# VisualComputingInstitute/diffusion-e2e-ft

Measured on NVIDIA H100. Metric: images_per_sec_768x768_depth, higher is better.
Workload: dtype fp16

## Files before the change

diffusion_e2e_ft_b200/build.py:

```python
import hashlib
import os
import subprocess
import sys
from concurrent.futures import ThreadPoolExecutor

HERE = os.path.dirname(os.path.abspath(__file__))
CSRC = os.path.join(HERE, "csrc")
OUT = os.path.join(HERE, "libb200_e2eft.so")
OBJ = os.path.join(HERE, "build")
SOURCES = ["gemm_conv.cu", "attention.cu", "norm.cu", "elementwise.cu", "conv_small.cu", "loss.cu", "optim.cu", "backward.cu", "postproc.cu",
           "evaluation.cu", "data.cu"]
NVCC = os.environ.get("NVCC", "/usr/local/cuda/bin/nvcc")
FLAGS = ["-gencode", "arch=compute_90a,code=sm_90a", "-O3", "-lineinfo", "-std=c++17",
         "-Xcompiler", "-fPIC"]


def _digest():
    h = hashlib.sha256()
    for root in (CSRC, os.path.join(HERE, "..", "include")):
        for f in sorted(os.listdir(root)):
            if f.endswith((".cu", ".cuh", ".h")):
                h.update(open(os.path.join(root, f), "rb").read())
    h.update(" ".join(FLAGS).encode())
    return h.hexdigest()


def build(force=False, verbose=False):
    os.makedirs(OBJ, exist_ok=True)
    stamp = os.path.join(OBJ, "stamp")
    dg = _digest()
    if not force and os.path.exists(OUT) and os.path.exists(stamp) and open(stamp).read() == dg:
        return OUT
    if not os.path.exists(NVCC):
        raise RuntimeError(f"nvcc not found at {NVCC}; cannot build {OUT}")

    def cc(src):
        obj = os.path.join(OBJ, src.replace(".cu", ".o"))
        cmd = [NVCC, *FLAGS, "-c", os.path.join(CSRC, src), "-o", obj]
        if verbose:
            cmd.insert(1, "-Xptxas=-v")
        r = subprocess.run(cmd, capture_output=True, text=True)
        if r.returncode != 0:
            raise RuntimeError(f"nvcc failed for {src}:\n{r.stdout}\n{r.stderr}")
        if verbose:
            print(r.stderr)
        return obj

    with ThreadPoolExecutor(max_workers=4) as ex:
        objs = list(ex.map(cc, SOURCES))
    r = subprocess.run([NVCC, "-shared", "-o", OUT, *objs, "-lcudart"], capture_output=True, text=True)
    if r.returncode != 0:
        raise RuntimeError(f"link failed:\n{r.stdout}\n{r.stderr}")
    open(stamp, "w").write(dg)
    return OUT


if __name__ == "__main__":
    print(build(force="--force" in sys.argv, verbose="-v" in sys.argv))
```

diffusion_e2e_ft_b200/csrc/gemm_conv.cu:

```cuda
#include <cstdarg>
#include <cstdio>
#include <cstring>
#include <mutex>

#include "gemm_conv.cuh"
#include "../../include/b200_e2eft.h"

namespace b200 {

static thread_local char g_err[512] = "";
void set_last_error(const char* fmt, ...) {
  va_list ap;
  va_start(ap, fmt);
  vsnprintf(g_err, sizeof(g_err), fmt, ap);
  va_end(ap);
}
const char* last_error() { return g_err; }

typedef CUresult (*EncodeTiledFn)(CUtensorMap*, CUtensorMapDataType, cuuint32_t, void*,
                                  const cuuint64_t*, const cuuint64_t*, const cuuint32_t*,
                                  const cuuint32_t*, CUtensorMapInterleave, CUtensorMapSwizzle,
                                  CUtensorMapL2promotion, CUtensorMapFloatOOBfill);
static EncodeTiledFn get_encode() {
  static EncodeTiledFn fn = nullptr;
  static std::once_flag once;
  std::call_once(once, [] {
    void* p = nullptr;
    cudaDriverEntryPointQueryResult q;
    if (cudaGetDriverEntryPoint("cuTensorMapEncodeTiled", &p, cudaEnableDefault, &q) == cudaSuccess &&
        q == cudaDriverEntryPointSuccess)
      fn = reinterpret_cast<EncodeTiledFn>(p);
  });
  return fn;
}

int encode_tmap(CUtensorMap* out, const void* gptr, int rank, const uint64_t* dims,
                const uint64_t* strides_bytes, const uint32_t* box, const uint32_t* elem_strides,
                CUtensorMapDataType dtype) {
  EncodeTiledFn fn = get_encode();
  if (!fn) {
    set_last_error("cuTensorMapEncodeTiled entry point unavailable (no CUDA driver?)");
    return -2;
  }
  cuuint64_t d[5], s[4];
  cuuint32_t b[5], e[5];
  for (int i = 0; i < rank; ++i) {
    d[i] = dims[i];
    b[i] = box[i];
    e[i] = elem_strides ? elem_strides[i] : 1;
  }
  for (int i = 0; i < rank - 1; ++i) s[i] = strides_bytes[i];
  CUresult r = fn(out, dtype, (cuuint32_t)rank, const_cast<void*>(gptr), d, s, b, e,
                  CU_TENSOR_MAP_INTERLEAVE_NONE, CU_TENSOR_MAP_SWIZZLE_128B,
                  CU_TENSOR_MAP_L2_PROMOTION_L2_256B, CU_TENSOR_MAP_FLOAT_OOB_FILL_NONE);
  if (r != CUDA_SUCCESS) {
    set_last_error(
        "cuTensorMapEncodeTiled failed (%d): rank %d dims [%llu %llu %llu %llu] strides [%llu %llu %llu] "
        "box [%u %u %u %u] ptr %p",
        (int)r, rank, (unsigned long long)d[0], (unsigned long long)(rank > 1 ? d[1] : 0),
        (unsigned long long)(rank > 2 ? d[2] : 0), (unsigned long long)(rank > 3 ? d[3] : 0),
        (unsigned long long)s[0], (unsigned long long)(rank > 2 ? s[1] : 0),
        (unsigned long long)(rank > 3 ? s[2] : 0), b[0], rank > 1 ? b[1] : 0, rank > 2 ? b[2] : 0,
        rank > 3 ? b[3] : 0, gptr);
    return -3;
  }
  return 0;
}

int current_device() {
  int dev = 0;
  return cudaGetDevice(&dev) == cudaSuccess && dev >= 0 && dev < kMaxDevices ? dev : -1;
}

int sm_count() {
  static int n[kMaxDevices] = {0};
  const int dev = current_device();
  if (dev < 0) return 132;
  if (!n[dev]) {
    int v = 0;
    cudaDeviceGetAttribute(&v, cudaDevAttrMultiProcessorCount, dev);
    n[dev] = v > 0 ? v : 132;
  }
  return n[dev];
}

constexpr int kLastLaunchFields = 16;
static int g_last_launch[kLastLaunchFields] = {0};

template <int BN, typename OutT, bool SWAP, bool GEGLU = false, bool HALO = false, bool VEC = false>
static int launch_one(const CUtensorMap& a, const CUtensorMap& a2, const CUtensorMap& b,
                      const GemmParams& p, cudaStream_t st) {
  using S = GemmSmem<BN, SWAP, HALO>;
  static bool configured_dev[kMaxDevices] = {false};
  const int dev = current_device();
  bool& configured = configured_dev[dev < 0 ? 0 : dev];
  auto kern = gemm_conv_kernel<BN, OutT, SWAP, GEGLU, HALO, VEC>;
  if (!configured || dev < 0) {
    cudaError_t e = cudaFuncSetAttribute(kern, cudaFuncAttributeMaxDynamicSharedMemorySize, S::kTotalBytes);
    if (e != cudaSuccess) {
      set_last_error("cudaFuncSetAttribute(smem=%d): %s", S::kTotalBytes, cudaGetErrorString(e));
      return (int)e;
    }
    configured = true;
  }
  int tiles = p.batch * p.m_tiles * p.n_tiles;
  int grid = tiles < sm_count() ? tiles : sm_count();
  if (SWAP && p.chan_stats && p.n_tiles > 1 && grid > p.n_tiles) grid -= grid % p.n_tiles;
  {
    const int rec[kLastLaunchFields] = {p.conv, HALO, SWAP, BN, VEC, GEGLU, (int)std::is_same<OutT, float>::value,
                                        p.bw, p.bh, p.halo_n, p.tiles_w, p.tiles_h, p.m_tiles, p.n_tiles, grid,
                                        p.chan_stats != nullptr};
    memcpy(g_last_launch, rec, sizeof(rec));
  }
  kern<<<grid, kGemmThreads, S::kTotalBytes, st>>>(a, a2, b, p);
  B200_CHECK_LAUNCH("gemm_conv_kernel");
  return 0;
}

template <typename OutT>
static int launch_bn(int bn, bool swap, const CUtensorMap& a, const CUtensorMap& a2, const CUtensorMap& b,
                     const GemmParams& p, cudaStream_t st) {
  if (swap) {
    switch (bn) {
      case 64: return p.vec_ok ? launch_one<64, OutT, true, false, false, true>(a, a2, b, p, st)
                               : launch_one<64, OutT, true>(a, a2, b, p, st);
      case 128: return p.vec_ok ? launch_one<128, OutT, true, false, false, true>(a, a2, b, p, st)
                                : launch_one<128, OutT, true>(a, a2, b, p, st);
      case 256: return p.vec_ok ? launch_one<256, OutT, true, false, false, true>(a, a2, b, p, st)
                                : launch_one<256, OutT, true>(a, a2, b, p, st);
    }
  } else if (p.act == ACT_GEGLU) {
    if constexpr (std::is_same<OutT, __half>::value) {
      switch (bn) {
        case 64: return launch_one<64, OutT, false, true>(a, a2, b, p, st);
        case 128: return launch_one<128, OutT, false, true>(a, a2, b, p, st);
        case 160: return launch_one<160, OutT, false, true>(a, a2, b, p, st);
        case 256: return launch_one<256, OutT, false, true>(a, a2, b, p, st);
      }
    }
    set_last_error("GEGLU epilogue needs fp16 output and a tile width in {64,128,160,256} (got %d)", bn);
    return -1;
  } else {
    switch (bn) {
      case 32: return launch_one<32, OutT, false>(a, a2, b, p, st);
      case 64: return launch_one<64, OutT, false>(a, a2, b, p, st);
      case 128: return launch_one<128, OutT, false>(a, a2, b, p, st);
      case 160: return launch_one<160, OutT, false>(a, a2, b, p, st);
      case 256: return launch_one<256, OutT, false>(a, a2, b, p, st);
    }
  }
  set_last_error("unsupported tile width %d (swap=%d)", bn, (int)swap);
  return -1;
}

static double kblock_cycles(int n) { return n * 4.0 > 365.0 ? n * 4.0 : 365.0; }
static double tiles_cost(long long tiles, int n) {
  long long waves = (tiles + sm_count() - 1) / sm_count();
  return (double)waves * (kblock_cycles(n) + 40.0);
}

static int g_force_bn = 0;
static int g_debug = 0;
static int g_swap_mode = 1;
static int g_halo_mode = 1;
static int g_last_path = 0;

static bool pick_halo_tile(int Ho, int Wo, int* bw_out, int* bh_out) {
  double best = 0.0;
  int bbw = 0, bbh = 0;
  for (int bw = 8; bw <= 254 && bw <= Wo; ++bw) {
    for (int bh = 1; bh <= 32 && bh <= Ho; ++bh) {
      const int pitch = bw + 2;
      const int n = (pitch * bh + 63) / 64 * 64;
      if (n > 256) break;
      if ((bh + 2) * pitch + (n - pitch * bh) + 2 > kHaloMaxPatchPix) continue;
      const double ew = (double)Wo / ((double)((Wo + bw - 1) / bw) * bw);
      const double eh = (double)Ho / ((double)((Ho + bh - 1) / bh) * bh);
      double score = ew * eh * (double)(bw * bh) / n;
      score *= 0.9 + 0.1 * n / 256.0;
      score *= 1.0 - 0.03 * ((double)(bw + 2) * (bh + 2) / (bw * bh) - 1.0);
      if (score > best + 1e-9) { best = score; bbw = bw; bbh = bh; }
    }
  }
  *bw_out = bbw; *bh_out = bbh;
  return bbw != 0 && best >= 0.78;
}

}

using namespace b200;

extern "C" const char* b200_last_error_string(void) { return b200::last_error(); }
extern "C" void b200_debug_force_block_n(int bn) { b200::g_force_bn = bn; }
extern "C" void b200_debug_set_flags(int f) { b200::g_debug = f; }
extern "C" void b200_debug_set_swap(int m) { b200::g_swap_mode = m; }
extern "C" void b200_debug_set_halo(int m) { b200::g_halo_mode = m; }
extern "C" int b200_debug_last_path(void) { return b200::g_last_path; }
extern "C" int b200_debug_last_launch(int* out, int n) {
  if (!out || n <= 0) return kLastLaunchFields;
  const int k = n < kLastLaunchFields ? n : kLastLaunchFields;
  memcpy(out, b200::g_last_launch, k * sizeof(int));
  return kLastLaunchFields;
}
extern "C" int b200_abi_version(void) { return 17; }
extern "C" int b200_geglu_block_n(int N) {
  return (N % 160 == 0) ? 160 : (N % 256 == 0 ? 256 : (N % 128 == 0 ? 128 : (N % 64 == 0 ? 64 : 0)));
}

extern "C" int b200_linear(const void* A, long long lda, long long a_batch_stride, const void* W,
                           long long ldw, long long w_batch_stride, int M, int N, int K, int batch,
                           const float* bias, int bias_row, const void* residual, long long ld_res,
                           long long res_batch_stride, void* out, long long ldo,
                           long long out_batch_stride, int out_f32, int act, float alpha,
                           double* chan_stats, int rows_per_img, void* out2_f16, int res_mul, int a_mn, int w_mn,
                           long long bias_batch_stride, void* stream) {
  B200_CHECK_ARG(A && W && out, "b200_linear: null pointer");
  B200_CHECK_ARG(!(a_mn || w_mn) || act != ACT_GEGLU, "b200_linear: MN-major operands are not combined with GEGLU");
  B200_CHECK_ARG(M > 0 && N > 0 && K > 0 && batch > 0, "b200_linear: bad shape M=%d N=%d K=%d batch=%d", M, N, K, batch);
  B200_CHECK_ARG(lda % 8 == 0 && ldw % 8 == 0, "b200_linear: lda/ldw must be multiples of 8 elements (16 B)");
  B200_CHECK_ARG(((uintptr_t)A & 15) == 0 && ((uintptr_t)W & 15) == 0 && ((uintptr_t)out & 15) == 0,
                 "b200_linear: pointers must be 16-byte aligned");
  B200_CHECK_ARG(act != ACT_GEGLU || ldo % 8 == 0, "b200_linear: GEGLU needs ldo %% 8 == 0");
  B200_CHECK_ARG(act != ACT_GEGLU || (N % 16 == 0 && bias), "b200_linear: GEGLU needs bias and N%%16==0");
  B200_CHECK_ARG(batch == 1 || (a_batch_stride % 8 == 0 && (w_batch_stride % 8 == 0)),
                 "b200_linear: batch strides must be multiples of 8 elements");

  B200_CHECK_ARG(!chan_stats || (batch == 1 && rows_per_img > 0 && rows_per_img % 64 == 0 && M % rows_per_img == 0 &&
                                 act != ACT_GEGLU && !bias_row),
                 "b200_linear: chan_stats needs batch=1, rows_per_img %% 64 == 0, M %% rows_per_img == 0");
  B200_CHECK_ARG((long long)M * ldo < 0xFFFFFFFFll && (long long)M * (ld_res > 0 ? ld_res : 1) < 0xFFFFFFFFll,
                 "b200_linear: per-batch output larger than 2^32 elements");
  GemmParams p;
  memset(&p, 0, sizeof(p));
  p.M = M; p.N = N;
  p.num_k_blocks = (K + kBlockK - 1) / kBlockK;
  p.batch = batch;
  p.m_tiles = (M + kBlockM - 1) / kBlockM;
  p.a_batched = (a_batch_stride != 0 && batch > 1);
  p.b_batched = (w_batch_stride != 0 && batch > 1);
  const bool can_swap = g_swap_mode && N >= 128 && act != ACT_GEGLU && !bias_row;
  bool swap = false;
  int bn = 0;
  double best = 1e30;
  if (act == ACT_GEGLU) {
    bn = b200_geglu_block_n(N);
    B200_CHECK_ARG(bn != 0, "b200_linear: GEGLU N=%d not tileable", N);
  } else {
    const int nc[5] = {256, 160, 128, 64, 32};
    const bool normal_ok = !chan_stats || rows_per_img % kBlockM == 0;
    for (int i = 0; i < 5 && normal_ok; ++i) {
      if (g_force_bn && nc[i] != g_force_bn) continue;
      if (w_mn && nc[i] % 64 != 0) continue;
      double c = tiles_cost((long long)p.m_tiles * batch * ((N + nc[i] - 1) / nc[i]), nc[i]);
      if (c < best - 1e-9) { best = c; bn = nc[i]; swap = false; }
    }
    if (can_swap || (chan_stats && !normal_ok && N >= 128)) {
      const int pc[3] = {256, 128, 64};
      for (int i = 0; i < 3; ++i) {
        if (g_force_bn && pc[i] != g_force_bn) continue;
        if (chan_stats && rows_per_img % pc[i] != 0) continue;
        if (a_mn && pc[i] % 64 != 0) continue;
        double c = tiles_cost((long long)batch * ((M + pc[i] - 1) / pc[i]) * ((N + 127) / 128), pc[i]) * 0.85;
        if (c < best - 1e-9) { best = c; bn = pc[i]; swap = true; }
      }
    }
    B200_CHECK_ARG(bn != 0, "b200_linear: no tile shape for N=%d (forced %d)", N, g_force_bn);
  }
  if (swap) {
    p.m_tiles = (M + bn - 1) / bn;
    p.n_tiles = (N + 127) / 128;
  } else {
    p.n_tiles = (N + bn - 1) / bn;
  }
  p.out = out; p.ldo = ldo; p.out_batch_stride = out_batch_stride; p.out_f32 = out_f32;
  p.bias = bias; p.bias_row = bias_row;
  p.residual = residual; p.ld_res = ld_res; p.res_batch_stride = res_batch_stride; p.res_mul = res_mul;
  p.act = act; p.alpha = alpha; p.debug = g_debug;
  p.chan_stats = chan_stats; p.rows_per_img = rows_per_img; p.out2 = (__half*)out2_f16;
  p.act_mn = a_mn; p.w_mn = w_mn;
  p.bias_bs = bias_batch_stride;
  p.out_mul = 1;
  {
    const uintptr_t omask = out_f32 ? 15 : 7;
    p.vec_ok = swap && (chan_stats != nullptr || (g_debug & 128)) && !(g_debug & 64) && N % 4 == 0 && ldo % 4 == 0 &&
               out_batch_stride % 4 == 0 && ((uintptr_t)out & omask) == 0 &&
               (!residual || (ld_res % 4 == 0 && res_batch_stride % 4 == 0 && ((uintptr_t)residual & omask) == 0)) &&
               (!out2_f16 || ((uintptr_t)out2_f16 & 7) == 0);
  }

  CUtensorMap ta, tb;
  if (a_mn) {
    uint64_t dims[3] = {(uint64_t)M, (uint64_t)K, (uint64_t)(p.a_batched ? batch : 1)};
    uint64_t str[2] = {(uint64_t)lda * 2, (uint64_t)(p.a_batched ? a_batch_stride : (long long)K * lda) * 2};
    uint32_t box[3] = {64, kBlockK, 1};
    int r = encode_tmap(&ta, A, 3, dims, str, box, nullptr);
    if (r) return r;
  } else {
    uint64_t dims[3] = {(uint64_t)K, (uint64_t)M, (uint64_t)(p.a_batched ? batch : 1)};
    uint64_t str[2] = {(uint64_t)lda * 2, (uint64_t)(p.a_batched ? a_batch_stride : (long long)M * lda) * 2};
    uint32_t box[3] = {kBlockK, (uint32_t)(swap ? bn : kBlockM), 1};
    int r = encode_tmap(&ta, A, 3, dims, str, box, nullptr);
    if (r) return r;
  }
  if (w_mn) {
    uint64_t dims[3] = {(uint64_t)N, (uint64_t)K, (uint64_t)(p.b_batched ? batch : 1)};
    uint64_t str[2] = {(uint64_t)ldw * 2, (uint64_t)(p.b_batched ? w_batch_stride : (long long)K * ldw) * 2};
    uint32_t box[3] = {64, kBlockK, 1};
    int r = encode_tmap(&tb, W, 3, dims, str, box, nullptr);
    if (r) return r;
  } else {
    uint64_t dims[3] = {(uint64_t)K, (uint64_t)N, (uint64_t)(p.b_batched ? batch : 1)};
    uint64_t str[2] = {(uint64_t)ldw * 2, (uint64_t)(p.b_batched ? w_batch_stride : (long long)N * ldw) * 2};
    uint32_t box[3] = {kBlockK, (uint32_t)(swap ? kBlockM : bn), 1};
    int r = encode_tmap(&tb, W, 3, dims, str, box, nullptr);
    if (r) return r;
  }
  cudaStream_t st = (cudaStream_t)stream;
  return out_f32 ? launch_bn<float>(bn, swap, ta, ta, tb, p, st) : launch_bn<__half>(bn, swap, ta, ta, tb, p, st);
}

static double pick_patch(int Ho, int Wo, int stride, int target, int* bw_out, int* bh_out) {
  double best = -1;
  int bbw = 1, bbh = 1;
  for (int bw = 1; bw <= target && bw <= Wo; ++bw) {
    if (bw * stride > 256) break;
    int bh = target / bw;
    if (bh > Ho) bh = Ho;
    if (bh * stride > 256) bh = 256 / stride;
    if (bh < 1) continue;
    long long tw = (Wo + bw - 1) / bw, th = (Ho + bh - 1) / bh;
    double eff = (double)Ho * Wo / (double)(tw * th * target);
    if (eff > best + 1e-9 || (eff > best - 1e-9 && bw > bbw)) {
      best = eff; bbw = bw; bbh = bh;
    }
  }
  *bw_out = bbw; *bh_out = bbh;
  return best;
}

extern "C" int b200_conv2d_nhwc(const void* X, int NB, int H, int W, int Cin, const void* X2, int C2,
                                const void* Wp, int Cout, int num_taps, const int* tap_dy,
                                const int* tap_dx, int stride, int Ho, int Wo, int out_mul, int out_oy,
                                int out_ox, const float* bias, const float* rowvec,
                                long long ld_rowvec, const void* residual, void* out, int out_f32,
                                int out_nchw, int act, double* chan_stats, void* out2_f16, void* stream) {
  B200_CHECK_ARG(X && Wp && out, "b200_conv2d_nhwc: null pointer");
  B200_CHECK_ARG(Cin % 64 == 0, "b200_conv2d_nhwc: Cin=%d must be a multiple of 64 (use im2col path)", Cin);
  B200_CHECK_ARG(C2 % 64 == 0, "b200_conv2d_nhwc: C2=%d must be a multiple of 64", C2);
  B200_CHECK_ARG(num_taps >= 1 && num_taps <= kMaxTaps, "b200_conv2d_nhwc: num_taps=%d", num_taps);
  B200_CHECK_ARG(stride >= 1 && stride <= 2 && out_mul >= 1, "b200_conv2d_nhwc: stride=%d out_mul=%d", stride, out_mul);
  B200_CHECK_ARG(NB > 0 && H > 0 && W > 0 && Ho > 0 && Wo > 0 && Cout > 0, "b200_conv2d_nhwc: bad shape");
  B200_CHECK_ARG(((uintptr_t)X & 15) == 0 && ((uintptr_t)Wp & 15) == 0 && ((uintptr_t)out & 15) == 0,
                 "b200_conv2d_nhwc: pointers must be 16-byte aligned");
  B200_CHECK_ARG(act != ACT_GEGLU, "b200_conv2d_nhwc: GEGLU epilogue is linear-only");
  B200_CHECK_ARG(!out_nchw || (!residual && Cout <= 8), "b200_conv2d_nhwc: out_nchw needs Cout <= 8 and no residual");

  B200_CHECK_ARG((long long)NB * Ho * out_mul * Wo * out_mul * Cout < 0xFFFFFFFFll,
                 "b200_conv2d_nhwc: output larger than 2^32 elements");
  GemmParams p;
  memset(&p, 0, sizeof(p));
  p.conv = 1;
  p.N = Cout;
  p.batch = 1;
  p.Ho = Ho; p.Wo = Wo;
  const bool can_swap = g_swap_mode && Cout >= 128 && !out_nchw;
  {
    bool taps_ok = stride == 1 && Ho == H && Wo == W && !(X2 && out_mul != 1);
    for (int i = 0; i < num_taps && taps_ok; ++i)
      taps_ok = tap_dy[i] >= -1 && tap_dy[i] <= 1 && tap_dx[i] >= -1 && tap_dx[i] <= 1;
    int hbw = 0, hbh = 0;
    const bool epi_bound = out_f32 && residual && num_taps * Cin <= 1152 && !X2;
    const bool halo_vec = !(g_debug & 64) && (Cout % 4 == 0) && (!residual || ((uintptr_t)residual & 15) == 0) &&
                          (!out2_f16 || ((uintptr_t)out2_f16 & 7) == 0);
    if (can_swap && g_halo_mode && taps_ok && !g_force_bn && halo_vec && (!epi_bound || g_halo_mode == 2) &&
        pick_halo_tile(Ho, Wo, &hbw, &hbh)) {
      p.bw = hbw; p.bh = hbh;
      p.col_pitch = hbw + 2;
      p.halo_n = ((hbw + 2) * hbh + 63) / 64 * 64;
      p.tiles_w = (Wo + hbw - 1) / hbw;
      p.tiles_h = (Ho + hbh - 1) / hbh;
      p.m_tiles = NB * p.tiles_w * p.tiles_h;
      p.n_tiles = (Cout + 127) / 128;
      p.M = NB * Ho * Wo;
      p.cin_blocks = Cin / 64;
// ... 129 lines not shown
```

diffusion_e2e_ft_b200/lib.py:

```python
import ctypes
import os
from ctypes import c_char_p, c_double, c_float, c_int, c_longlong, c_void_p, POINTER

_HERE = os.path.dirname(os.path.abspath(__file__))
LIB_PATH = os.path.join(_HERE, "libb200_e2eft.so")

_lib = None
ABI_VERSION = 17

_P = c_void_p
_LL = c_longlong
_SIGS = {
    "b200_last_error_string": (c_char_p, []),
    "b200_abi_version": (c_int, []),
    "b200_debug_force_block_n": (None, [c_int]),
    "b200_debug_set_flags": (None, [c_int]),
    "b200_debug_set_swap": (None, [c_int]),
    "b200_debug_set_halo": (None, [c_int]),
    "b200_debug_last_path": (c_int, []),
    "b200_debug_last_launch": (c_int, [POINTER(c_int), c_int]),
    "b200_geglu_block_n": (c_int, [c_int]),
    "b200_linear": (c_int, [_P, _LL, _LL, _P, _LL, _LL, c_int, c_int, c_int, c_int, _P, c_int, _P, _LL, _LL,
                            _P, _LL, _LL, c_int, c_int, c_float, _P, c_int, _P, c_int, c_int, c_int, _LL, _P]),
    "b200_conv2d_nhwc": (c_int, [_P, c_int, c_int, c_int, c_int, _P, c_int, _P, c_int, c_int,
                                 POINTER(c_int), POINTER(c_int), c_int, c_int, c_int, c_int, c_int, c_int,
                                 _P, _P, _LL, _P, _P, c_int, c_int, c_int, _P, _P, _P]),
    "b200_conv3x3_small_cout": (c_int, [_P, c_int, c_int, c_int, c_int, _P, _P, c_int, _P, _P]),
    "b200_im2col3x3_nchw": (c_int, [_P, c_int, c_int, c_int, c_int, c_int, _P, c_int, _P]),
    "b200_group_norm_stats": (c_int, [_P, c_int, _P, c_int, c_int, c_int, c_int, c_int, _P, _P]),
    "b200_group_norm_apply": (c_int, [_P, c_int, _P, c_int, c_int, c_int, c_int, c_int, _P, _P, _P, c_float,
                                      c_int, _P, _P, _P]),
    "b200_group_norm_apply_cs": (c_int, [_P, c_int, _P, _P, c_int, _P, c_int, c_int, c_int, c_int, _P, _P, c_float,
                                         c_int, _P, _P, _P]),
    "b200_layer_norm": (c_int, [_P, c_int, _LL, c_int, _P, _P, c_float, _P, _P]),
    "b200_attention": (c_int, [_P, _LL, _LL, _P, _LL, _LL, _P, _LL, _LL, _P, _LL, _LL, c_int, c_int, c_int, c_int,
                               c_int, c_int, c_float, _P, _P]),
    "b200_attention_d64": (c_int, [_P, _LL, _LL, _P, _LL, _LL, _P, _LL, _LL, _P, _LL, _LL, c_int, c_int, c_int,
                                   c_int, c_int, c_float, _P, _P]),
    "b200_attention_d512": (c_int, [_P, _LL, _LL, _P, _LL, _LL, _P, _LL, _LL, _P, _LL, _LL, c_int, c_int, c_int,
                                    c_float, _P]),
    "b200_rowdot_heads_d": (c_int, [_P, _LL, _LL, _P, _LL, _LL, c_int, c_int, c_int, c_int, _P, _P]),
    "b200_rowdot_heads": (c_int, [_P, _LL, _LL, _P, _LL, _LL, c_int, c_int, c_int, _P, _P]),
    "b200_softmax_rows": (c_int, [_P, _LL, _P, _LL, _LL, c_int, c_float, _P]),
    "b200_softmax_groups": (c_int, [_P, c_int, _LL, c_int, c_int, _P, c_int, _P]),
    "b200_upsample_nearest_nhwc": (c_int, [_P, c_int, c_int, c_int, c_int, c_int, c_int, c_int, _P, _P]),
    "b200_timestep_embedding": (c_int, [_P, c_int, c_int, _P, _P]),
    "b200_embed_tokens": (c_int, [_P, _P, _P, c_int, _LL, c_int, c_int, c_int, _P, _P]),
    "b200_pointwise_nchw": (c_int, [_P, c_float, _P, c_float, c_int, _P, _P, c_int, c_int, c_int, _LL, _P, _P]),
    "b200_decode_post": (c_int, [_P, c_int, _LL, c_int, c_float, _P, _P]),
    "b200_ddim_step": (c_int, [_P, c_int, _LL, _P, _LL, c_int, c_int, _LL, c_int, c_float, c_float, _P, _P, _P, c_int,
                               _LL, _P]),
    "b200_ssi_loss": (c_int, [_P, _P, _P, c_int, _LL, _P, _P, _P]),
    "b200_angular_loss": (c_int, [_P, _P, _P, c_int, _LL, _P, _P, _P]),
    "b200_sumsq": (c_int, [_P, _LL, _P, _P]),
    "b200_adamw_step": (c_int, [_P, _P, _P, _P, _LL, c_float, c_float, c_float, c_float, c_float, c_int, _P,
                                c_float, _P]),
    "b200_gather_planar": (c_int, [_P, c_int, _LL, c_int, c_int, c_int, c_int, c_int, c_int, c_int, c_int, c_int, c_int, _P,
                                   _LL, _P]),
    "b200_col_sum": (c_int, [_P, c_int, _LL, c_int, _LL, _P, _P]),
    "b200_group_norm_mean_rstd": (c_int, [_P, _P, c_int, _P, c_int, c_int, c_int, c_int, c_float, _P, _P]),
    "b200_group_norm_bwd_sums": (c_int, [_P, c_int, c_int, c_int, c_int, _P, c_int, c_int, c_int, _P, _P, _P, c_int,
                                         _P, _P]),
    "b200_group_norm_bwd_apply": (c_int, [_P, c_int, c_int, c_int, c_int, _P, c_int, c_int, c_int, _P, _P, _P, c_int,
                                          _P, _P, _P, c_int, _P]),
    "b200_layer_norm_bwd": (c_int, [_P, c_int, _LL, c_int, _P, _P, c_float, _P, _P, c_int, _P, _P, _P]),
    "b200_softmax_bwd_rows": (c_int, [_P, _LL, _P, _LL, _P, _LL, c_int, c_float, _P]),
    "b200_act_bwd": (c_int, [_P, _P, _LL, c_int, _P, _P]),
    "b200_geglu_bwd": (c_int, [_P, _P, _LL, _P, _LL, c_int, _P, _P, _LL, _P]),
    "b200_ssi_loss_bwd": (c_int, [_P, _P, _P, c_int, _LL, _P, _P, _P, _P]),
    "b200_angular_loss_bwd": (c_int, [_P, _P, _P, c_int, _LL, _P, _P, _P, _P]),
    "b200_decode_post_bwd": (c_int, [_P, _P, c_int, _LL, c_int, _P, _P]),
    "b200_adamw_step_scaled": (c_int, [_P, _P, _P, _P, _LL, c_float, c_float, c_float, c_float, c_float, c_int, _P,
                                       c_float, c_float, _P]),
    "b200_adamw_step_state": (c_int, [_P, _P, _P, _P, _LL, c_float, c_float, c_float, c_float, c_float, _P, c_float,
                                      c_float, _P, c_int, c_float, c_float, c_float, _P]),
    "b200_adamw_step_state_groups": (c_int, [_P, _P, _P, _P, _LL, _P, _P, c_int, _P, _P, c_int, c_float, c_float,
                                             c_float, _P, c_float, c_float, _P, c_int, c_float, c_float, c_float, _P]),
    "b200_upsample_nearest_bwd": (c_int, [_P, c_int, c_int, c_int, c_int, c_int, c_int, _P, _P, _P]),
    "b200_ensemble_normals": (c_int, [_P, c_int, _LL, _P, _P, _P, _P]),
    "b200_ensemble_depths_objective": (c_int, [_P, _P, _P, c_int, _LL, c_int, _P, _P, _P]),
    "b200_ensemble_depths_reduce": (c_int, [_P, _P, _P, c_int, _LL, c_int, _P, _P, _P, _P]),
    "b200_minmax_rows": (c_int, [_P, c_int, _LL, _P, _P, _P]),
    "b200_minmax_normalise": (c_int, [_P, _LL, _P, _P, _P]),
    "b200_rgb_normalise": (c_int, [_P, c_int, _LL, c_int, _P, _P]),
    "b200_resize_bilinear_aa": (c_int, [_P, _LL, c_int, c_int, c_int, c_int, _P, _P, _P]),
    "b200_resize_bicubic_aa": (c_int, [_P, _LL, c_int, c_int, c_int, c_int, _P, _P, _P]),
    "b200_resize_nearest": (c_int, [_P, _LL, c_int, c_int, c_int, c_int, _P, _P]),
    "b200_resize_nearest_exact": (c_int, [_P, _LL, c_int, c_int, c_int, c_int, _P, _P]),
    "b200_colorize_depth": (c_int, [_P, _LL, _P, c_int, _P, _P]),
    "b200_colorize_normals": (c_int, [_P, _LL, _P, _P]),
    "b200_diffusion_inputs": (c_int, [_P, _P, _P, _P, _P, c_int, c_int, _LL, c_int, _P, _P, _P]),
    "b200_masked_latent_mse": (c_int, [_P, c_int, _P, _P, c_int, c_int, c_int, c_int, c_int, c_int, _P, _P, _P, _P]),
    "b200_masked_latent_mse_bwd": (c_int, [_P, c_int, _P, _P, _P, _P, c_int, c_int, _LL, _P, _P]),
    "b200_ema_update": (c_int, [_P, _P, _LL, c_float, _P]),
    "b200_cast_f32_to_f16": (c_int, [_P, _P, _LL, _P]),
    "b200_nhwc_to_nchw_f32": (c_int, [_P, c_int, c_int, c_int, _LL, _P, _P]),
    "b200_eval_align_depth": (c_int, [_P, _P, _P, c_int, c_int, c_int, c_int, c_float, c_int, _P, _P, _P]),
    "b200_eval_depth_metrics": (c_int, [_P, _P, _P, c_int, _LL, _P, c_int, c_int, c_float, c_float, _P, _P, _P, _P]),
    "b200_eval_normal_error": (c_int, [_P, POINTER(c_longlong), _P, POINTER(c_longlong), _P, c_int, c_int, c_int, _P,
                                       _P, _LL, _P, _P, _P, _P, _P]),
    "b200_eval_kth_smallest": (c_int, [_P, _P, _LL, _LL, _P, _P, _P]),
    "b200_data_hypersim_source": (c_int, [_P, _P, _P, c_int, c_int, c_int, POINTER(c_double), _P, _P, _P]),
    "b200_data_resize_u8": (c_int, [_P, c_int, c_int, c_int, c_int, c_int, c_int, _P, _P, c_int, _P, _P, c_int, _P, _P,
                                    _P, _P]),
    "b200_data_depth_gather": (c_int, [_P, _P, c_int, c_int, c_int, c_int, c_int, _P, _P, _P, _P, _P]),
    "b200_data_depth_range": (c_int, [_P, c_int, _LL, c_float, c_float, _P, _P, _P]),
    "b200_data_finalise": (c_int, [_P, _P, c_int, c_int, c_int, c_int, c_int, _P, _P, c_int, c_int, c_float, c_float,
                                   _P, _P, _P, _P, _P, _P, _P, _P]),
    "b200_data_vkitti_normals": (c_int, [_P, c_int, c_int, c_int, c_float, c_float, c_float, c_float, _P, _P]),
    "b200_debug_pow_e32_neg": (c_int, [_P, _LL, c_int, _P, _P, _P]),
    "b200_data_hypersim_workspace_bytes": (_LL, [c_int, c_int, c_int]),
    "b200_data_hypersim_frames": (c_int, [_P, c_int, _P, c_int, _P, c_int, c_int, c_int, c_double, c_double, _P, _P, _P,
                                          _P, _P, _LL, _P]),
    "b200_debug_hypersim_pow": (c_int, [_P, _LL, c_int, _P, _P, _P, _P]),
}
EXPORTS = tuple(_SIGS)


def load(build_if_missing=True):
    global _lib
    if _lib is not None:
        return _lib
    from . import build as _build
    if not os.path.exists(LIB_PATH) and not build_if_missing:
        raise RuntimeError(f"{LIB_PATH} is missing — run `python -m diffusion_e2e_ft_b200.build`")
    if build_if_missing and os.path.exists(_build.NVCC):
        _build.build()
    elif not os.path.exists(LIB_PATH):
        raise RuntimeError(f"{LIB_PATH} is missing and nvcc is not available to build it")
    lib = ctypes.CDLL(LIB_PATH)
    lib.b200_abi_version.restype = c_int
    if lib.b200_abi_version() != ABI_VERSION:
        raise RuntimeError(f"{LIB_PATH} exports ABI {lib.b200_abi_version()}, this package binds ABI {ABI_VERSION}: "
                           "rebuild with `python -m diffusion_e2e_ft_b200.build --force`")
    for name, (res, args) in _SIGS.items():
        fn = getattr(lib, name)
        fn.restype = res
        fn.argtypes = args
    _lib = lib
    return lib


def check(rc, what):
    if rc != 0:
        msg = load().b200_last_error_string()
        raise RuntimeError(f"{what} failed (rc={rc}): {msg.decode() if msg else '?'}")
```

include/b200_e2eft.h:

```cpp
#ifndef B200_E2EFT_H_
#define B200_E2EFT_H_

#ifdef __cplusplus
extern "C" {
#endif

const char* b200_last_error_string(void);
int b200_abi_version(void);

#define B200_ACT_NONE 0
#define B200_ACT_SILU 1
#define B200_ACT_GEGLU 2
#define B200_ACT_GELU 3
#define B200_ACT_EXP2 4

int b200_linear(const void* A, long long lda, long long a_batch_stride,
                const void* W, long long ldw, long long w_batch_stride ,
                int M, int N, int K, int batch,
                const float* bias, int bias_row,
                const void* residual, long long ld_res, long long res_batch_stride,
                void* out, long long ldo, long long out_batch_stride, int out_f32,
                int act, float alpha,
                double* chan_stats ,
                int rows_per_img,
                void* out2_f16 ,
                int res_mul ,
                int a_mn ,
                int w_mn ,
                long long bias_batch_stride ,
                void* stream);

int b200_geglu_block_n(int N);

int b200_conv2d_nhwc(const void* X, int NB, int H, int W, int Cin,
                     const void* X2, int C2,
                     const void* Wp, int Cout, int num_taps, const int* tap_dy, const int* tap_dx,
                     int stride, int Ho, int Wo, int out_mul, int out_oy, int out_ox,
                     const float* bias, const float* rowvec, long long ld_rowvec,
                     const void* residual, void* out, int out_f32, int out_nchw, int act,
                     double* chan_stats ,
                     void* out2_f16 , void* stream);

int b200_conv3x3_small_cout(const void* x, int NB, int H, int W, int C, const void* wq,
                            const float* bias, int Cout, float* out, void* stream);

int b200_im2col3x3_nchw(const void* x, int x_f32, int NB, int C, int H, int W, void* out,
                        int Kpad, void* stream);

int b200_group_norm_stats(const void* x1, int C1, const void* x2, int C2, int in_f32, int NB,
                          int HW, int groups, double* sums, void* stream);
int b200_group_norm_apply(const void* x1, int C1, const void* x2, int C2, int in_f32, int NB, int HW,
                          int groups, const double* sums, const float* gamma, const float* beta,
                          float eps, int silu, void* y, void* raw_copy, void* stream);

int b200_group_norm_apply_cs(const void* x1, int C1, const double* cs1, const void* x2, int C2,
                             const double* cs2, int in_f32, int NB, int HW, int groups,
                             const float* gamma, const float* beta, float eps, int silu, void* y,
                             void* raw_copy, void* stream);

int b200_layer_norm(const void* x, int in_f32, long long rows, int C, const float* gamma,
                    const float* beta, float eps, void* y, void* stream);

int b200_attention(const void* q, long long q_bs, long long q_ls,
                   const void* k, long long k_bs, long long k_ls,
                   const void* v, long long v_bs, long long v_ls,
                   void* out, long long o_bs, long long o_ls,
                   int B, int heads, int head_dim, int Lq, int Lk, int kv_segments, float scale,
                   float* lse ,
                   void* stream);
int b200_attention_d64(const void* q, long long q_bs, long long q_ls,
                       const void* k, long long k_bs, long long k_ls,
                       const void* v, long long v_bs, long long v_ls,
                       void* out, long long o_bs, long long o_ls,
                       int B, int heads, int Lq, int Lk, int kv_segments, float scale, float* lse, void* stream);

int b200_attention_d512(const void* q, long long q_bs, long long q_ls,
                        const void* k, long long k_bs, long long k_ls,
                        const void* v, long long v_bs, long long v_ls,
                        void* out, long long o_bs, long long o_ls,
                        int B, int Lq, int Lk, float scale, void* stream);

int b200_softmax_rows(const float* S, long long lds, void* P, long long ldp, long long rows,
                      int cols, float scale, void* stream);

int b200_softmax_groups(const float* logits, int ld_in, long long rows, int heads, int S, void* P, int ld_out,
                        void* stream);

int b200_upsample_nearest_nhwc(const void* x, int in_f32, int NB, int H, int W, int C, int OH,
                               int OW, void* y, void* stream);

int b200_timestep_embedding(const float* t, int B, int dim, void* out, void* stream);

int b200_embed_tokens(const long long* ids, const void* tok, const void* pos, int w_f32, long long rows, int L, int C,
                      int vocab, float* out, void* stream);

int b200_pointwise_nchw(const float* in1, float a1, const float* in2, float a2, int in_cstride,
                        const float* Wm, const float* bias, int NB, int Cin, int Cout, long long HW,
                        float* out, void* stream);

#define B200_PRED_EPSILON 0
#define B200_PRED_V 1
#define B200_PRED_SAMPLE 2
int b200_ddim_step(const void* model_out, int mo_f16, long long mo_bstride, const float* sample, long long s_bstride,
                   int B, int C, long long HW, int prediction_type, float alpha_prod_t, float alpha_prod_t_prev,
                   float* prev_sample, float* pred_original_sample, void* unet_in, int unet_in_f16,
                   long long ui_bstride, void* stream);

int b200_decode_post(const float* x, int NB, long long HW, int mode, float sign, float* out,
                     void* stream);

int b200_ssi_loss(const float* pred, const float* target, const unsigned char* mask, int B, long long HW,
                  double* workspace, float* out, void* stream);
int b200_angular_loss(const float* pred, const float* target, const unsigned char* mask, int B, long long HW,
                      double* workspace, float* out, void* stream);

int b200_sumsq(const float* x, long long n, double* out, void* stream);
int b200_adamw_step(float* param, const float* grad, float* exp_avg, float* exp_avg_sq, long long n,
                    float lr, float beta1, float beta2, float eps, float weight_decay, int step,
                    const double* grad_norm_sq, float max_grad_norm, void* stream);
int b200_adamw_step_scaled(float* param, const float* grad, float* exp_avg, float* exp_avg_sq, long long n,
                           float lr, float beta1, float beta2, float eps, float weight_decay, int step,
                           const double* grad_norm_sq, float max_grad_norm, float grad_unscale, void* stream);

int b200_adamw_step_state(float* param, const float* grad, float* exp_avg, float* exp_avg_sq, long long n,
                          float lr, float beta1, float beta2, float eps, float weight_decay,
                          const double* grad_norm_sq, float max_grad_norm, float inv_world, float* state,
                          int dynamic_scale, float growth_interval, float min_scale, float max_scale, void* stream);

#define B200_ADAMW_MAX_GROUPS 16
#define B200_ADAMW_MAX_RUNS 1024
int b200_adamw_step_state_groups(float* param, const float* grad, float* exp_avg, float* exp_avg_sq, long long n,
                                 const long long* run_start, const int* run_group, int n_runs, const float* group_lr,
                                 const float* group_wd, int n_groups, float beta1, float beta2, float eps,
                                 const double* grad_norm_sq, float max_grad_norm, float inv_world, float* state,
                                 int dynamic_scale, float growth_interval, float min_scale, float max_scale,
                                 void* stream);

int b200_gather_planar(const void* x, int in_f32, long long ldx, int NB, int H, int W, int C, int Ho, int Wo, int stride, int up,
                       int oy, int ox, void* out, long long ldo, void* stream);
int b200_col_sum(const void* x, int in_f32, long long rows, int C, long long ld, float* out, void* stream);
int b200_rowdot_heads_d(const void* a, long long a_bs, long long a_ls, const void* c, long long c_bs, long long c_ls,
                        int B, int L, int heads, int head_dim, float* out, void* stream);
int b200_rowdot_heads(const void* a, long long a_bs, long long a_ls, const void* c, long long c_bs, long long c_ls,
                      int B, int L, int heads, float* out, void* stream);
int b200_group_norm_mean_rstd(const double* sums, const double* cs1, int C1, const double* cs2, int C2, int NB, int HW,
                              int groups, float eps, float* mean_rstd, void* stream);
int b200_group_norm_bwd_sums(const void* x, int in_f32, int Cx, int c_off, int Ctot, const void* dy, int NB, int HW,
                             int groups, const float* mean_rstd, const float* gamma, const float* beta, int silu,
                             float* S, void* stream);
int b200_group_norm_bwd_apply(const void* x, int in_f32, int Cx, int c_off, int Ctot, const void* dy, int NB, int HW,
                              int groups, const float* mean_rstd, const float* gamma, const float* beta, int silu,
                              const float* S, const void* add, void* dx, int out_f32, void* stream);
int b200_layer_norm_bwd(const void* x, int in_f32, long long rows, int C, const float* gamma, const void* dy,
                        float eps, const void* add, void* dx, int out_f32, float* dgamma, float* dbeta, void* stream);
int b200_softmax_bwd_rows(const void* P, long long ldp, const float* dP, long long ldd, void* dS, long long rows,
                          int cols, float scale, void* stream);
int b200_act_bwd(const void* x, const void* dy, long long n, int act, void* dx, void* stream);
int b200_geglu_bwd(const void* h, const void* g, long long ld_hg, const void* dy, long long rows, int inner, void* dh,
                   void* dg, long long ld_d, void* stream);

int b200_ssi_loss_bwd(const float* pred, const float* target, const unsigned char* mask, int B, long long HW,
                      double* workspace, const float* grad_out, float* dpred, void* stream);
int b200_angular_loss_bwd(const float* pred, const float* target, const unsigned char* mask, int B, long long HW,
                          double* workspace, const float* grad_out, float* dpred, void* stream);
int b200_decode_post_bwd(const float* x, const float* dout, int NB, long long HW, int mode, float* dx, void* stream);
int b200_upsample_nearest_bwd(const float* dy, int NB, int H, int W, int C, int OH, int OW, const float* add,
                              float* dx, void* stream);

int b200_cast_f32_to_f16(const float* x, void* y, long long n, void* stream);
int b200_nhwc_to_nchw_f32(const void* x, int in_f32, int NB, int C, long long HW, float* y, void* stream);

void b200_debug_force_block_n(int bn);
void b200_debug_set_flags(int flags);
void b200_debug_set_swap(int mode);
void b200_debug_set_halo(int mode);
int b200_debug_last_path(void);
int b200_debug_last_launch(int* out, int n);

int b200_resize_bicubic_aa(const float* x, long long planes, int H, int W, int OH, int OW, float* tmp, float* out,
                           void* stream);

int b200_ensemble_normals(const float* preds, int E, long long HW, double* err_ws, float* out, int* index, void* stream);
int b200_ensemble_depths_objective(const float* imgs, const float* s, const float* t, int E, long long HW,
                                   int reduction, double* ws, float* out3, void* stream);
int b200_ensemble_depths_reduce(const float* imgs, const float* s, const float* t, int E, long long HW, int reduction,
                                double* ws, float* aligned, float* uncertainty, void* stream);
int b200_minmax_rows(const float* x, int rows, long long cols, unsigned int* ws, float* out, void* stream);
int b200_minmax_normalise(float* x, long long n, unsigned int* ws, float* minmax_out, void* stream);
int b200_rgb_normalise(const void* x, int in_u8, long long n, int round_u8, float* out, void* stream);
int b200_resize_bilinear_aa(const float* x, long long planes, int H, int W, int OH, int OW, float* tmp, float* out,
                            void* stream);
int b200_resize_nearest(const float* x, long long planes, int H, int W, int OH, int OW, float* out, void* stream);

int b200_resize_nearest_exact(const float* x, long long planes, int H, int W, int OH, int OW, float* out, void* stream);
int b200_colorize_depth(const float* x, long long n, const unsigned char* table, int ncol, unsigned char* out,
                        void* stream);
int b200_colorize_normals(const float* x, long long HW, unsigned char* out, void* stream);

int b200_diffusion_inputs(const float* rgb_latents, const float* x0, const float* noise, const long long* timesteps,
                          const float* alphas_cumprod, int B, int C, long long HW, int prediction_type, float* unet_in,
                          float* target, void* stream);
int b200_masked_latent_mse(const void* pred, int pred_f16, const float* target, const unsigned char* val_mask, int B,
                           int C, int H, int W, int h, int w, unsigned char* latent_mask, double* workspace, float* out,
                           void* stream);
int b200_masked_latent_mse_bwd(const void* pred, int pred_f16, const float* target, const unsigned char* latent_mask,
                               const double* workspace, const float* grad_out, int B, int C, long long hw, void* grad,
                               void* stream);
int b200_ema_update(float* ema, const float* param, long long n, float one_minus_decay, void* stream);

#define B200_EVAL_MAX_BLOCKS 512
#define B200_EVAL_KTH_WS_WORDS 261
int b200_eval_align_depth(const float* gt, const float* pred, const unsigned char* mask, int B, int H, int W, int OW,
                          float col_scale, int disparity, double* ws, float* scale_shift, void* stream);
int b200_eval_depth_metrics(const float* pred, const float* gt, const unsigned char* mask, int B, long long HW,
                            const float* scale_shift, int disparity, int clip, float min_depth, float max_depth,
                            float* aligned, double* ws, float* out, void* stream);
int b200_eval_normal_error(const float* pred, const long long* pred_strides, const float* gt,
                           const long long* gt_strides, const unsigned char* mask, int B, int H, int W, float* err_map,
                           float* buf, long long buf_capacity, unsigned long long* buf_len, double* ws, double* sums,
                           long long* counts, void* stream);
int b200_eval_kth_smallest(const float* x, const unsigned long long* n, long long n_max, long long k,
                           unsigned long long* ws, float* out, void* stream);

int b200_data_hypersim_source(const unsigned short* depth_mm, const unsigned char* normal, const unsigned char* flip,
                              int B, int H, int W, const double* inv_k, float* depth_m, unsigned char* normal_out,
                              void* stream);
int b200_data_resize_u8(const unsigned char* src, int B, int H, int W, int C, int OH, int OW, const int* xmin,
                        const int* xk, int xks, const int* ymin, const int* yk, int yks, const unsigned char* flip,
                        unsigned char* tmp, unsigned char* dst, void* stream);
int b200_data_depth_gather(const float* src_m, const unsigned short* src_cm, int B, int H, int W, int OH, int OW,
                           const int* rows, const int* cols, const unsigned char* flip, float* dst, void* stream);
int b200_data_depth_range(const float* depth, int B, long long HW, float near_plane, float far_plane, float* range,
                          int* flag, void* stream);
int b200_data_finalise(const unsigned char* rgb, const unsigned char* normal, int B, int H, int W, int top, int left,
                       const unsigned char* flip, const float* depth, int OH, int OW, float near_plane,
                       float far_plane, const float* range, const int* flag, float* rgb_out, float* depth_out,
                       float* metric_out, float* normal_out, unsigned char* mask_out, void* stream);

int b200_data_vkitti_normals(const unsigned short* depth_cm, int B, int H, int W, float fx, float fy, float u0,
                             float v0, unsigned short* out, void* stream);
int b200_debug_pow_e32_neg(const float* x, long long n, int force_slow, float* out, unsigned int* slow_count,
                           void* stream);

long long b200_data_hypersim_workspace_bytes(int B, int H, int W);
int b200_data_hypersim_frames(const void* rgb, int rgb_half, const void* dist, int dist_half, const int* entity_id,
                              int B, int H, int W, double focal, double scale_num, unsigned char* bgr,
                              unsigned short* depth_mm, int* error_flag, double* stats_out, void* workspace,
                              long long workspace_bytes, void* stream);
int b200_debug_hypersim_pow(const double* x, long long n, int force_slow, double* p_out, unsigned char* level_out,
                            unsigned int* slow_count, void* stream);

#ifdef __cplusplus
}
#endif
#endif
```

Baseline: 40.61.

## Add persistent ping-pong linear GEMM kernel overlapping epilogue with mainloop

Adds a persistent warp-specialized linear GEMM kernel in which two consumer warpgroups alternate tiles. Named barriers order them so one warpgroup's epilogue (bias, residual, activation, stores) runs while the other issues WGMMA on the next tile. It also uses a deeper TMA stage ring and prefetches residual rows into L2. The kernel is used only for large batch-1 linears with moderate aspect ratios and simple activations; other cases fall back to the existing path. The risks are that each warpgroup holds a full 128xBN accumulator in registers, and that the pipeline bookkeeping across tiles adds complexity.

```diff
diff --git a/diffusion_e2e_ft_b200/build.py b/diffusion_e2e_ft_b200/build.py
--- a/diffusion_e2e_ft_b200/build.py
+++ b/diffusion_e2e_ft_b200/build.py
@@ -8,7 +8,7 @@
 CSRC = os.path.join(HERE, "csrc")
 OUT = os.path.join(HERE, "libb200_e2eft.so")
 OBJ = os.path.join(HERE, "build")
-SOURCES = ["gemm_conv.cu", "attention.cu", "norm.cu", "elementwise.cu", "conv_small.cu", "loss.cu", "optim.cu", "backward.cu", "postproc.cu",
+SOURCES = ["gemm_conv.cu", "gemm_linear.cu", "attention.cu", "norm.cu", "elementwise.cu", "conv_small.cu", "loss.cu", "optim.cu", "backward.cu", "postproc.cu",
            "evaluation.cu", "data.cu"]
 NVCC = os.environ.get("NVCC", "/usr/local/cuda/bin/nvcc")
 FLAGS = ["-gencode", "arch=compute_90a,code=sm_90a", "-O3", "-lineinfo", "-std=c++17",
diff --git a/diffusion_e2e_ft_b200/csrc/gemm_conv.cu b/diffusion_e2e_ft_b200/csrc/gemm_conv.cu
--- a/diffusion_e2e_ft_b200/csrc/gemm_conv.cu
+++ b/diffusion_e2e_ft_b200/csrc/gemm_conv.cu
@@ -3,7 +3,7 @@
 #include <cstring>
 #include <mutex>
 
-#include "gemm_conv.cuh"
+#include "gemm_linear.cuh"
 #include "../../include/b200_e2eft.h"
 
 namespace b200 {
@@ -164,6 +164,8 @@
 static int g_swap_mode = 1;
 static int g_halo_mode = 1;
 static int g_last_path = 0;
+static int g_overlap_mode = 1;
+static int g_last_linear = 0;
 
 static bool pick_halo_tile(int Ho, int Wo, int* bw_out, int* bh_out) {
   double best = 0.0;
@@ -196,6 +198,8 @@
 extern "C" void b200_debug_set_swap(int m) { b200::g_swap_mode = m; }
 extern "C" void b200_debug_set_halo(int m) { b200::g_halo_mode = m; }
 extern "C" int b200_debug_last_path(void) { return b200::g_last_path; }
+extern "C" void b200_debug_set_linear_overlap(int m) { b200::g_overlap_mode = m; }
+extern "C" int b200_debug_last_linear_kernel(void) { return b200::g_last_linear; }
 extern "C" int b200_debug_last_launch(int* out, int n) {
   if (!out || n <= 0) return kLastLaunchFields;
   const int k = n < kLastLaunchFields ? n : kLastLaunchFields;
@@ -230,6 +234,16 @@
                  "b200_linear: chan_stats needs batch=1, rows_per_img %% 64 == 0, M %% rows_per_img == 0");
   B200_CHECK_ARG((long long)M * ldo < 0xFFFFFFFFll && (long long)M * (ld_res > 0 ? ld_res : 1) < 0xFFFFFFFFll,
                  "b200_linear: per-batch output larger than 2^32 elements");
+  g_last_linear = 0;
+  if (g_overlap_mode && !g_force_bn && !g_debug && batch == 1 && !a_mn && !w_mn && act != ACT_GEGLU && !chan_stats &&
+      !bias_row) {
+    const int r = linear_overlap(A, lda, W, ldw, M, N, K, bias, residual, ld_res, out, ldo, out_f32, act, alpha,
+                                 out2_f16, res_mul, (cudaStream_t)stream);
+    if (r != 1) {
+      g_last_linear = 1;
+      return r;
+    }
+  }
   GemmParams p;
   memset(&p, 0, sizeof(p));
   p.M = M; p.N = N;
diff --git a/diffusion_e2e_ft_b200/csrc/gemm_linear.cu b/diffusion_e2e_ft_b200/csrc/gemm_linear.cu
--- /dev/null
+++ b/diffusion_e2e_ft_b200/csrc/gemm_linear.cu
@@ -0,0 +1,66 @@
+#include "gemm_linear.cuh"
+
+namespace b200 {
+
+template <int BN, typename OutT>
+static int launch_linear(const CUtensorMap& ta, const CUtensorMap& tb, const LinearParams& p, cudaStream_t st) {
+  using S = LinearSmem<BN>;
+  static bool configured_dev[kMaxDevices] = {false};
+  const int dev = current_device();
+  bool& configured = configured_dev[dev < 0 ? 0 : dev];
+  auto kern = linear_overlap_kernel<BN, OutT>;
+  if (!configured || dev < 0) {
+    cudaError_t e = cudaFuncSetAttribute(kern, cudaFuncAttributeMaxDynamicSharedMemorySize, S::kTotalBytes);
+    if (e != cudaSuccess) {
+      set_last_error("cudaFuncSetAttribute(smem=%d): %s", S::kTotalBytes, cudaGetErrorString(e));
+      return (int)e;
+    }
+    configured = true;
+  }
+  const int tiles = p.m_tiles * p.n_tiles;
+  const int grid = tiles < sm_count() ? tiles : sm_count();
+  kern<<<grid, kGemmThreads, S::kTotalBytes, st>>>(ta, tb, p);
+  B200_CHECK_LAUNCH("linear_overlap_kernel");
+  return 0;
+}
+
+int linear_overlap(const void* A, long long lda, const void* W, long long ldw, int M, int N, int K, const float* bias,
+                   const void* residual, long long ld_res, void* out, long long ldo, int out_f32, int act, float alpha,
+                   void* out2_f16, int res_mul, cudaStream_t st) {
+  const int bn = (N % 128 != 0 && N % 160 == 0) ? 160 : 128;
+  const long long m_tiles = (M + kBlockM - 1) / kBlockM, n_tiles = (N + bn - 1) / bn;
+  if (m_tiles * n_tiles < 2LL * sm_count()) return 1;
+  if (N >= 4LL * K || K >= 4LL * N) return 1;
+  if (act != ACT_NONE && act != ACT_SILU && act != ACT_GELU) return 1;
+  if (N % 8 != 0 || ldo % 8 != 0 || ((uintptr_t)out & 15) != 0) return 1;
+  if (residual && (ld_res % 8 != 0 || ((uintptr_t)residual & 15) != 0)) return 1;
+  if (bias && ((uintptr_t)bias & 7) != 0) return 1;
+  if (out2_f16 && (!out_f32 || ((uintptr_t)out2_f16 & 15) != 0)) return 1;
+
+  LinearParams p;
+  p.M = M; p.N = N;
+  p.num_k_blocks = (K + kBlockK - 1) / kBlockK;
+  p.m_tiles = (int)m_tiles; p.n_tiles = (int)n_tiles;
+  p.out = out; p.ldo = ldo; p.bias = bias;
+  p.residual = residual; p.ld_res = ld_res; p.res_mul = res_mul;
+  p.act = act; p.alpha = alpha; p.out2 = (__half*)out2_f16;
+  CUtensorMap ta, tb;
+  {
+    uint64_t dims[3] = {(uint64_t)K, (uint64_t)M, 1};
+    uint64_t str[2] = {(uint64_t)lda * 2, (uint64_t)M * lda * 2};
+    uint32_t box[3] = {kBlockK, kBlockM, 1};
+    int r = encode_tmap(&ta, A, 3, dims, str, box, nullptr);
+    if (r) return r;
+  }
+  {
+    uint64_t dims[3] = {(uint64_t)K, (uint64_t)N, 1};
+    uint64_t str[2] = {(uint64_t)ldw * 2, (uint64_t)N * ldw * 2};
+    uint32_t box[3] = {kBlockK, (uint32_t)bn, 1};
+    int r = encode_tmap(&tb, W, 3, dims, str, box, nullptr);
+    if (r) return r;
+  }
+  if (bn == 160) return out_f32 ? launch_linear<160, float>(ta, tb, p, st) : launch_linear<160, __half>(ta, tb, p, st);
+  return out_f32 ? launch_linear<128, float>(ta, tb, p, st) : launch_linear<128, __half>(ta, tb, p, st);
+}
+
+}
diff --git a/diffusion_e2e_ft_b200/csrc/gemm_linear.cuh b/diffusion_e2e_ft_b200/csrc/gemm_linear.cuh
--- /dev/null
+++ b/diffusion_e2e_ft_b200/csrc/gemm_linear.cuh
@@ -0,0 +1,213 @@
+#pragma once
+#include "gemm_conv.cuh"
+
+namespace b200 {
+
+struct LinearParams {
+  int M, N, num_k_blocks, m_tiles, n_tiles;
+  void* out;
+  long long ldo;
+  const float* bias;
+  const void* residual;
+  long long ld_res;
+  int res_mul;
+  int act;
+  float alpha;
+  __half* out2;
+};
+
+template <int BN>
+struct LinearSmem {
+  static constexpr int kABytes = kBlockM * kBlockK * 2;
+  static constexpr int kBBytes = BN * kBlockK * 2;
+  static constexpr int kStageBytes = kABytes + kBBytes;
+  static constexpr int kBarrierBytes = 256;
+  static constexpr int kStages = (227 * 1024 - 1024  - kBarrierBytes) / kStageBytes;
+  static constexpr int kTotalBytes = kStages * kStageBytes + kBarrierBytes + 1024;
+  static_assert(kBBytes % 1024 == 0, "SWIZZLE_128B tiles start on 1024-byte boundaries");
+  static_assert(2 * kStages * 8 <= kBarrierBytes && kTotalBytes <= 227 * 1024, "shared memory budget");
+};
+
+__device__ __forceinline__ void named_bar_sync(int id, int threads) {
+  asm volatile("bar.sync %0, %1;" ::"r"(id), "r"(threads) : "memory");
+}
+__device__ __forceinline__ void named_bar_arrive(int id, int threads) {
+  asm volatile("bar.arrive %0, %1;" ::"r"(id), "r"(threads) : "memory");
+}
+
+template <typename OutT>
+__device__ __forceinline__ void load_pair(const OutT* src, float& a, float& b);
+template <>
+__device__ __forceinline__ void load_pair<float>(const float* src, float& a, float& b) {
+  const float2 v = *reinterpret_cast<const float2*>(src);
+  a = v.x; b = v.y;
+}
+template <>
+__device__ __forceinline__ void load_pair<__half>(const __half* src, float& a, float& b) {
+  const float2 v = __half22float2(*reinterpret_cast<const __half2*>(src));
+  a = v.x; b = v.y;
+}
+
+template <int BN, typename OutT>
+__global__ void __launch_bounds__(kGemmThreads, 1)
+linear_overlap_kernel(const __grid_constant__ CUtensorMap tmA, const __grid_constant__ CUtensorMap tmB,
+                      const LinearParams p) {
+  using S = LinearSmem<BN>;
+  constexpr int kStages = S::kStages;
+  constexpr int kHalf = BN / 2;
+  extern __shared__ __align__(16) uint8_t smem_raw[];
+  uint8_t* smem = smem_raw + ((1024u - (smem_u32(smem_raw) & 1023u)) & 1023u);
+  uint8_t* smem_a = smem;
+  uint8_t* smem_b = smem + kStages * S::kABytes;
+  uint64_t* full_bar = reinterpret_cast<uint64_t*>(smem + kStages * S::kStageBytes);
+  uint64_t* empty_bar = full_bar + kStages;
+
+  const int warp = threadIdx.x >> 5;
+  const int lane = threadIdx.x & 31;
+  const int total_tiles = p.m_tiles * p.n_tiles;
+
+  if (warp == kEpiWarps && lane == 0) {
+    tma_prefetch_desc(&tmA);
+    tma_prefetch_desc(&tmB);
+    for (int i = 0; i < kStages; ++i) {
+      mbar_init(&full_bar[i], 1);
+      mbar_init(&empty_bar[i], 128);
+    }
+    fence_barrier_init();
+  }
+  __syncthreads();
+
+  if (warp >= kEpiWarps) {
+    asm volatile("setmaxnreg.dec.sync.aligned.u32 %0;" ::"n"(kProducerRegs));
+    if (warp != kEpiWarps || lane != 0) return;
+    int stage = 0;
+    uint32_t phase = 0;
+    for (int tile = blockIdx.x; tile < total_tiles; tile += gridDim.x) {
+      const int n_blk = tile % p.n_tiles;
+      const int m_blk = tile / p.n_tiles;
+      for (int kb = 0; kb < p.num_k_blocks; ++kb) {
+        mbar_wait(&empty_bar[stage], phase ^ 1);
+        mbar_arrive_expect_tx(&full_bar[stage], (uint32_t)S::kStageBytes);
+        tma_load_3d(&tmA, &full_bar[stage], smem_a + stage * S::kABytes, kb * kBlockK, m_blk * kBlockM, 0, kEvictNormal);
+        tma_load_3d(&tmB, &full_bar[stage], smem_b + stage * S::kBBytes, kb * kBlockK, n_blk * BN, 0, kEvictLast);
+        if (++stage == kStages) { stage = 0; phase ^= 1; }
+      }
+    }
+    return;
+  }
+
+  asm volatile("setmaxnreg.inc.sync.aligned.u32 %0;" ::"n"(kConsumerRegs));
+  const int wg = warp >> 2;
+  const int wl = warp & 3;
+  OutT* __restrict__ out = reinterpret_cast<OutT*>(p.out);
+  const OutT* __restrict__ res = reinterpret_cast<const OutT*>(p.residual);
+  const float* __restrict__ bias = p.bias;
+  const uint32_t a_base = smem_u32(smem_a), b_base = smem_u32(smem_b);
+  float d[BN];
+
+  for (int it = wg, tile = blockIdx.x + wg * gridDim.x; tile < total_tiles; it += 2, tile += 2 * gridDim.x) {
+    const long long pos = (long long)it * p.num_k_blocks;
+    int stage = (int)(pos % kStages);
+    uint32_t phase = (uint32_t)((pos / kStages) & 1);
+    const int n_blk = tile % p.n_tiles;
+    const int m_blk = tile / p.n_tiles;
+    if (res != nullptr) {
+      const int row = m_blk * kBlockM + (threadIdx.x & 127);
+      const int bytes = min(BN, p.N - n_blk * BN) * (int)sizeof(OutT);
+      if (row < p.M) {
+        const char* src = reinterpret_cast<const char*>(res + (long long)row * p.ld_res + n_blk * BN);
+        for (int off = 0; off < bytes; off += 128) asm volatile("prefetch.global.L2 [%0];" ::"l"(src + off));
+      }
+    }
+    if (it > 0) named_bar_sync(1 + wg, 256);
+#pragma unroll
+    for (int i = 0; i < BN; ++i) d[i] = 0.f;
+    int prev = -1;
+    for (int kb = 0; kb < p.num_k_blocks; ++kb) {
+      mbar_wait(&full_bar[stage], phase);
+      const uint64_t adesc = make_desc_sw128(a_base + stage * S::kABytes, 16, 1024);
+      const uint64_t bdesc = make_desc_sw128(b_base + stage * S::kBBytes, 16, 1024);
+      wgmma_fence_operands<BN>(d);
+      wgmma_fence();
+#pragma unroll
+      for (int k = 0; k < kBlockK / kMmaK; ++k) {
+        wgmma_n<BN, 0, 0>(d, adesc + 2 * k, bdesc + 2 * k, (kb | k) != 0);
+        wgmma_n<BN, 0, 0>(d + kHalf, adesc + 512 + 2 * k, bdesc + 2 * k, (kb | k) != 0);
+      }
+      wgmma_commit();
+      wgmma_fence_operands<BN>(d);
+      wgmma_wait<1>();
+      if (prev >= 0) mbar_arrive(&empty_bar[prev]);
+      prev = stage;
+      if (++stage == kStages) { stage = 0; phase ^= 1; }
+    }
+    if (tile + gridDim.x < total_tiles) named_bar_arrive(1 + (wg ^ 1), 256);
+    wgmma_wait<0>();
+    wgmma_fence_operands<BN>(d);
+    mbar_arrive(&empty_bar[prev]);
+
+    const int col0 = n_blk * BN + 2 * (lane & 3);
+#pragma unroll
+    for (int h = 0; h < 2; ++h) {
+#pragma unroll
+      for (int rr = 0; rr < 2; ++rr) {
+        asm volatile("" ::: "memory");
+        const int row = m_blk * kBlockM + 64 * h + 16 * wl + (lane >> 2) + 8 * rr;
+        if (row >= p.M) continue;
+        OutT* __restrict__ orow = out + (long long)row * p.ldo + col0;
+        const OutT* __restrict__ rrow = res ? res + (long long)row * p.ld_res + col0 : nullptr;
+        __half* __restrict__ o2row = p.out2 ? p.out2 + (long long)row * p.ldo + col0 : nullptr;
+        float r[BN / 4];
+        if (rrow != nullptr) {
+#pragma unroll
+          for (int j = 0; j < BN / 8; ++j)
+            if (col0 + 8 * j < p.N) load_pair<OutT>(rrow + 8 * j, r[2 * j], r[2 * j + 1]);
+        }
+        float v[BN / 4];
+#pragma unroll
+        for (int j = 0; j < BN / 8; ++j) {
+          float add0 = 0.f, add1 = 0.f;
+          if (bias && col0 + 8 * j < p.N) {
+            const float2 b2 = *reinterpret_cast<const float2*>(bias + col0 + 8 * j);
+            add0 += b2.x;
+            add1 += b2.y;
+          }
+          v[2 * j] = fmaf(d[h * kHalf + 4 * j + 2 * rr], p.alpha, add0);
+          v[2 * j + 1] = fmaf(d[h * kHalf + 4 * j + 2 * rr + 1], p.alpha, add1);
+        }
+        if (rrow != nullptr && !p.res_mul) {
+#pragma unroll
+          for (int e = 0; e < BN / 4; ++e) v[e] += r[e];
+        }
+        if (p.act == ACT_SILU) {
+#pragma unroll
+          for (int e = 0; e < BN / 4; ++e) v[e] = silu_f(v[e]);
+        } else if (p.act == ACT_GELU) {
+#pragma unroll
+          for (int e = 0; e < BN / 4; ++e) v[e] = gelu_erf_f(v[e]);
+        }
+        if (rrow != nullptr && p.res_mul) {
+#pragma unroll
+          for (int e = 0; e < BN / 4; ++e) v[e] *= r[e];
+        }
+#pragma unroll
+        for (int j = 0; j < BN / 8; ++j) {
+          if (col0 + 8 * j >= p.N) continue;
+          const __half2 hv = __floats2half2_rn(v[2 * j], v[2 * j + 1]);
+          if constexpr (std::is_same<OutT, float>::value) {
+            *reinterpret_cast<float2*>(orow + 8 * j) = make_float2(v[2 * j], v[2 * j + 1]);
+            if (o2row != nullptr) *reinterpret_cast<__half2*>(o2row + 8 * j) = hv;
+          } else {
+            *reinterpret_cast<__half2*>(orow + 8 * j) = hv;
+          }
+        }
+      }
+    }
+  }
+}
+
+int linear_overlap(const void* A, long long lda, const void* W, long long ldw, int M, int N, int K, const float* bias,
+                   const void* residual, long long ld_res, void* out, long long ldo, int out_f32, int act, float alpha,
+                   void* out2_f16, int res_mul, cudaStream_t st);
+
+}
diff --git a/diffusion_e2e_ft_b200/lib.py b/diffusion_e2e_ft_b200/lib.py
--- a/diffusion_e2e_ft_b200/lib.py
+++ b/diffusion_e2e_ft_b200/lib.py
@@ -19,6 +19,8 @@
     "b200_debug_set_halo": (None, [c_int]),
     "b200_debug_last_path": (c_int, []),
     "b200_debug_last_launch": (c_int, [POINTER(c_int), c_int]),
+    "b200_debug_set_linear_overlap": (None, [c_int]),
+    "b200_debug_last_linear_kernel": (c_int, []),
     "b200_geglu_block_n": (c_int, [c_int]),
     "b200_linear": (c_int, [_P, _LL, _LL, _P, _LL, _LL, c_int, c_int, c_int, c_int, _P, c_int, _P, _LL, _LL,
                             _P, _LL, _LL, c_int, c_int, c_float, _P, c_int, _P, c_int, c_int, c_int, _LL, _P]),
diff --git a/include/b200_e2eft.h b/include/b200_e2eft.h
--- a/include/b200_e2eft.h
+++ b/include/b200_e2eft.h
@@ -176,6 +176,8 @@
 void b200_debug_set_halo(int mode);
 int b200_debug_last_path(void);
 int b200_debug_last_launch(int* out, int n);
+void b200_debug_set_linear_overlap(int mode);
+int b200_debug_last_linear_kernel(void);
 
 int b200_resize_bicubic_aa(const float* x, long long planes, int H, int W, int OH, int OW, float* tmp, float* out,
                            void* stream);
```

Result: no change. 40.75, median of 6 (+0.4%).
